# CAMMA-public/SelfPose3d

Measured on AMD Instinct MI355X. Metric: multi-view samples/sec (5-view Panoptic, 80x80x20 voxel), higher is better.
Workload: dtype f32

## Files before the change

include/sp3d.h:

```cpp
#ifndef SP3D_H
#define SP3D_H

#include <stdint.h>

#ifdef __cplusplus
extern "C" {
#endif

#define SP3D_ABI_VERSION 3
#define SP3D_MAX_VIEWS 16
#define SP3D_MAX_TOPK 32

#define SP3D_CAM_STRIDE 64
#define SP3D_CAM_R 0
#define SP3D_CAM_T 9
#define SP3D_CAM_F 12
#define SP3D_CAM_C 14
#define SP3D_CAM_K 16
#define SP3D_CAM_P 19
#define SP3D_CAM_A 21
#define SP3D_CAM_W0 27
#define SP3D_CAM_H0 28
#define SP3D_CAM_FLIP 29
#define SP3D_CAM_RXY 32
// ... 119 lines not shown
                              float beta, void *stream);

int sp3d_channel_shift_act(float *y, const float *shift, const float *residual, int mode, int64_t batch, int C,
                           int64_t inner, int channels_last, void *stream);

int sp3d_fetch_ring(const float *ring, float *dst, uint32_t *counter, int R, int n, void *stream);

int sp3d_maxpool2x_cl(const float *x, float *y, int B, int X, int Y, int Z, int C, void *stream);

int sp3d_crop_shift_act_cl(const float *src, float *dst, const float *shift, int B, int C, int X, int Y, int Z, int SX, int SY,
                           int SZ, int relu, void *stream);

int sp3d_rfft3d(const float *in, float *out, int batch, int SX, int SY, int SZ, void *stream);
int sp3d_irfft3d(float *in, float *out, int batch, int SX, int SY, int SZ, void *stream);

int sp3d_cfft2d(float *data, int batch, int SX, int SY, int inverse, void *stream);
int sp3d_cfft2d_ex(float *data, int batch, int SX, int SY, int inverse, int rows_in, int rows_out, void *stream);

int sp3d_zdft_fwd_cl(const float *x, float *spec, int B, int C, int Cout, int X, int Y, int Z, int SX, int SY, int SZ,
                     void *stream);
int sp3d_zdft_inv_cl(const float *spec, float *y, const float *shift, int B, int O, int X, int Y, int Z, int SX, int SY, int SZ,
                     int relu, void *stream);

int sp3d_unproject_fwd_zdft(const float *const *hm_views, int Jp, const float *cam, const float *centers,
                            const uint8_t *valid, float *spec, int B, int V, int J, int h, int w, int X, int Y, int Z,
                            const float grid_size[3], int W_in, int H_in, int SZ, void *stream);
int sp3d_cfft2d_88_tiled(const float *tiled, float *planes, int batch, int X, int Y, void *stream);

int sp3d_freq_contract_ty(const float *X, const float *T, const float *tw, float *Y, int B, int C, int O, int rows, int SY,
                          void *stream);

int sp3d_gaussian_target_3d(const float *roots, int B, int R, const float *gx, const float *gy, const float *gz, int X,
                            int Y, int Z, float sigma, float *target, void *stream);
int sp3d_render_root_heatmaps(const float *roots, int B, int R, const float *cam, int V, int h, int w, float stride,
                              float *out, void *stream);
int sp3d_render_joints_fwd(const float *kps, const int *count, int N, int P, int J, int h, int w, float sigma, float *out,
                           void *stream);
int sp3d_render_joints_bwd(const float *kps, const int *count, const float *grad_out, int N, int P, int J, int h, int w,
                           float sigma, float *grad_kps, void *stream);

int sp3d_freq_contract(const float *X, const float *W, float *Y, int B, int C, int O, int64_t F, void *stream);
int sp3d_freq_contract_ex(const float *P, const float *Q, float *Y, int I, int J, int K, int64_t F, int64_t sPi,
                          int64_t sPk, int64_t sQj, int64_t sQk, int conj_p, int conj_q, void *stream);

int sp3d_wino_input(const float *x, float *V, int B, int X, int Y, int Z, int C, void *stream);
int sp3d_wino_output(const float *M, float *y, const float *shift, const float *residual, int mode, int B, int X, int Y,
                     int Z, int O, void *stream);
int sp3d_wino_fused(const float *x, const float *U, float *y, const float *shift, const float *residual, int mode, int B,
                    int X, int Y, int Z, int C, int O, void *stream);

int sp3d_wino_fused_split(const float *x, const void *U3, float *y, const float *shift, const float *residual, int mode, int B,
                          int X, int Y, int Z, int C, int O, void *stream);

int sp3d_wino_fused_split64(const float *x, const void *U3, float *y, const float *shift, const float *residual, int mode,
                            int B, int X, int Y, int Z, int C, int O, void *stream);

int sp3d_conv3_split(const float *x, const void *W3, float *y, const float *shift, const float *residual, int mode, int B,
                     int X, int Y, int Z, int C, int O, void *stream);


int sp3d_conv3_split_skip(const float *x, const void *W3, float *y, const float *shift, const float *xs, const void *WS,
                          int B, int X, int Y, int Z, int C, int O, int CS, void *stream);

int sp3d_wino_fused_split64_skip(const float *x, const void *U3, float *y, const float *shift, const float *xs, const void *WS,
                                 int B, int X, int Y, int Z, int C, int O, int CS, void *stream);

int sp3d_upsample2x_scatter(const float *G, float *out, const float *shift, const float *skip, int64_t batch, int X, int Y,
                            int Z, int O, void *stream);

int sp3d_upsample2x_scatter_head(const float *G, float *head, const float *shift, const float *skip, const float *wout,
                                 const float *bout, int64_t batch, int X, int Y, int Z, int O, int J, void *stream);

int sp3d_upconv2x_fused(const float *x, const void *w_split, const float *shift, const float *skip, const float *w_out,
                        const float *b_out, float *out, int64_t batch, int X, int Y, int Z, int CIN, int O, int J, void *stream);

#define SP3D_GBN_F32 0
#define SP3D_GBN_F64 1
#define SP3D_GBN_REPLICAS 16
#define SP3D_GBN_PLAIN 0
#define SP3D_GBN_RELU 1
#define SP3D_GBN_ADD_RELU 2
int64_t sp3d_gbn_workspace_bytes(int G, int C);
int sp3d_gbn_forward(const void *x, void *y, int dtype, const int32_t *group_of, const int32_t *group_samples, int N,
                     int64_t S, int C, int G, int G_update, const void *weight, const void *bias, void *running_mean,
                     void *running_var, double eps, double momentum, int mode, const void *residual, void *mean,
                     void *invstd, void *scale, void *shift, double *workspace, void *stream);
int sp3d_gbn_backward(const void *x, const void *dy, void *dx, int dtype, const int32_t *group_of,
                      const int32_t *group_samples, int N, int64_t S, int C, int G, const void *weight, const void *mean,
                      const void *invstd, const void *scale, const void *shift, int mode, const void *y,
                      void *grad_residual, void *grad_weight, void *grad_bias, void *k123, double *workspace, void *stream);

#ifdef __cplusplus
}
#endif
#endif
```

selfpose3d_amd/_lib.py:

```python
from __future__ import annotations

import ctypes as C
import os
from typing import Optional, Sequence

import torch

_HERE = os.path.dirname(os.path.abspath(__file__))
_DEFAULT_LIB_PATH = os.path.join(_HERE, "libsp3d.so")
NOPK_LIB_PATH = os.path.join(_HERE, "libsp3d_nopk.so")
LIB_PATH = os.environ.get("SP3D_LIB_PATH") or _DEFAULT_LIB_PATH

LAYOUT_PLANAR = 0
LAYOUT_NHWC = 1
OUT_CHANNELS_LAST = 0x100
HM_BF16 = 0x200
OUT_BF16 = 0x400
HM_ONE_CHANNEL = 0x800
HM_WIDE_MASK = 0x1000
OUT_ZSPECTRUM = 0x2000
HM_ONE_ZSPECTRUM = 0x4000
SCATTER_AUTO, SCATTER_PER_TAP, SCATTER_MERGE = 0, 2, 3
SCATTER_WIDE = 0x100
MAX_VIEWS = 16
MAX_TOPK = 32
ABI_VERSION = 3

_CTYPES = {"p": C.c_void_p, "i": C.c_int, "l": C.c_int64, "f": C.c_float, "d": C.c_double, "s": C.c_char_p}

SIGNATURES = {
    "sp3d_abi_version": "i:",
    "sp3d_camera_finish": "i: p i",
    "sp3d_error_string": "s: i",
    "sp3d_pack_heatmaps": "i: pp iiiiii p",
    "sp3d_pack_heatmaps_ex": "i: pp iiiiiiii p",
    "sp3d_unproject_fwd": "i: p ii ppppp iiiiiiii p ii p",
    "sp3d_unproject_fwd_indexed": "i: p ii pppppp iiiiiiii p ii p",
    "sp3d_unproject_fwd_strided": "i: p ii pppppp iiiiiiii p ii p",
    "sp3d_unproject_bwd": "i: pppppp iiiiiiii p ii p",
    "sp3d_unproject_bwd_indexed": "i: ppppppp iiiiiiii p ii p",
    "sp3d_unproject_fwd_train": "i: p ii ppppppp iiiiiiii p ii p",
    "sp3d_unproject_bwd_packed": "i: ppppppp iiiiiiiiii p iii p",
    "sp3d_unproject_bwd_packed_det": "i: pppppppp iiiiiiiiii p iii p",
    "sp3d_fixed_to_float": "i: ppp l p",
    "sp3d_unproject_one_fwd_train": "i: p ii ppppppp iiiiiiii p ii p",
    "sp3d_unproject_one_bwd": "i: ppppp l pp iiiiiiii p ii p",
    "sp3d_unproject_one_bwd_det": "i: ppppp l ppp iiiiiiii p ii p",
    "sp3d_nms_topk_workspace_bytes": "l: iiiii",
    "sp3d_nms_topk": "i: p iiiii ppppppp",
    "sp3d_nms_proposals": "i: p iiiii pp f pppppp",
    "sp3d_soft_argmax": "i: ppp ii l f p",
    "sp3d_soft_argmax_grid": "i: ppp iii p ii f p",
    "sp3d_soft_argmax_grid_train": "i: ppp iii pp ii f p",
    "sp3d_soft_argmax_grid_bwd": "i: ppp iii pppp ii f p",
    "sp3d_channel_shift_act": "i: ppp i l i l i p",
    "sp3d_fetch_ring": "i: ppp ii p",
    "sp3d_maxpool2x_cl": "i: pp iiiii p",
    "sp3d_crop_shift_act_cl": "i: ppp iiiiiiiii p",
    "sp3d_rfft3d": "i: pp iiii p",
    "sp3d_irfft3d": "i: pp iiii p",
    "sp3d_cfft2d": "i: p iiii p",
    "sp3d_cfft2d_ex": "i: p iiiiii p",
    "sp3d_zdft_fwd_cl": "i: pp iiiiiiiii p",
    "sp3d_zdft_inv_cl": "i: ppp iiiiiiiii p",
    "sp3d_unproject_fwd_zdft": "i: p i pppp iiiiiiii p iii p",
    "sp3d_cfft2d_88_tiled": "i: pp iii p",
    "sp3d_freq_contract_ty": "i: pppp iiiii p",
    "sp3d_gaussian_target_3d": "i: p ii ppp iii f pp",
    "sp3d_render_root_heatmaps": "i: p ii p iii f pp",
    "sp3d_render_joints_fwd": "i: pp iiiii f pp",
    "sp3d_render_joints_bwd": "i: ppp iiiii f pp",
    "sp3d_freq_contract": "i: ppp iii l p",
    "sp3d_freq_contract_ex": "i: ppp iii lllll ii p",
    "sp3d_wino_input": "i: pp iiiii p",
    "sp3d_wino_output": "i: pppp iiiiii p",
    "sp3d_wino_fused": "i: ppppp iiiiiii p",
# ... 716 lines not shown

def freq_contract_ex(Pf: torch.Tensor, Qf: torch.Tensor, mode: str, *, out: Optional[torch.Tensor] = None) -> torch.Tensor:
    lib = load()
    _require_cuda(Pf, "Pf")
    Pf, Qf = Pf.resolve_conj().contiguous(), Qf.resolve_conj().contiguous()
    if Pf.dtype != torch.complex64 or Qf.dtype != torch.complex64 or Pf.shape[2:] != Qf.shape[2:]:
        raise Sp3dError("freq_contract_ex: complex64 operands with equal frequency shape expected")
    Fn = 1
    for d in Pf.shape[2:]:
        Fn *= int(d)
    p0, p1, q0, q1 = int(Pf.shape[0]), int(Pf.shape[1]), int(Qf.shape[0]), int(Qf.shape[1])
    if mode == "fwd":
        I, K, J = p0, p1, q0
        sPi, sPk, sQj, sQk, cp, cq = p1 * Fn, Fn, q1 * Fn, Fn, 0, 1
        ok = q1 == p1
    elif mode == "dx":
        I, K, J = p0, p1, q1
        sPi, sPk, sQj, sQk, cp, cq = p1 * Fn, Fn, Fn, q1 * Fn, 0, 0
        ok = q0 == p1
    elif mode == "dw":
        I, K, J = p1, p0, q1
        sPi, sPk, sQj, sQk, cp, cq = Fn, p1 * Fn, Fn, q1 * Fn, 1, 0
        ok = q0 == p0
    else:
        raise Sp3dError(f"freq_contract_ex: unknown mode {mode}")
    if not ok:
        raise Sp3dError("freq_contract_ex: contracted dimensions differ")
    Y = _result_dense(out, (I, J) + tuple(Pf.shape[2:]), torch.complex64, Pf.device, "freq_contract_ex")
    check(lib.sp3d_freq_contract_ex(Pf.data_ptr(), Qf.data_ptr(), Y.data_ptr(), I, J, K, Fn, sPi, sPk, sQj, sQk, cp, cq,
                                    _stream(Pf.device)), "sp3d_freq_contract_ex")
    return Y


_WINO_G = ((1.0, 0.0, 0.0), (0.5, 0.5, 0.5), (0.5, -0.5, 0.5), (0.0, 0.0, 1.0))


def wino_weights(w: torch.Tensor) -> torch.Tensor:
    G = torch.tensor(_WINO_G, dtype=torch.float64, device=w.device)
    u = torch.einsum("ai,bj,ck,ozijk->abczo", G, G, G, w.double())
    return u.reshape(64, w.shape[1], w.shape[0]).float().contiguous()


def wino_weights_split(U: torch.Tensor, chunk: int = 8) -> torch.Tensor:
    P, Cc, O = (int(v) for v in U.shape)
    U = U.float()
    hi = U.bfloat16()
    r = U - hi.float()
    mid = r.bfloat16()
    lo = (r - mid.float()).bfloat16()
    pieces = torch.stack([mid, hi, lo], 0).reshape(3, P, Cc // chunk, chunk // 4, 4, O)
    return pieces.permute(1, 2, 3, 5, 0, 4).contiguous()


def conv_weights_split(w: torch.Tensor) -> torch.Tensor:
    O, Cc = int(w.shape[0]), int(w.shape[1])
    taps = int(w.shape[2]) * int(w.shape[3]) * int(w.shape[4])
    pc = wino_weights_split(w.float().permute(4, 3, 2, 1, 0).reshape(taps, Cc, O).contiguous(), 8)
    mid, hi, lo = pc[..., 0, :], pc[..., 1, :], pc[..., 2, :]
    return torch.stack([hi, lo, hi, hi, mid, mid], -2).contiguous()


def conv_weights_split24(w: torch.Tensor) -> torch.Tensor:
    O, Cc = int(w.shape[0]), int(w.shape[1])
    pc = wino_weights_split(w.float().permute(4, 3, 2, 1, 0).reshape(27, Cc, O).contiguous(), 8)
    pc = pc.reshape(27, Cc // 8, 2, O // 32, 32, 3, 4).permute(0, 1, 3, 2, 4, 5, 6)
    hl = torch.stack([pc[..., 1, :], pc[..., 2, :]], -2).reshape(27, Cc // 8, O // 32, 512)
    mid = pc[..., 0, :].reshape(27, Cc // 8, O // 32, 256)
    return torch.cat([hl, mid], -1).contiguous()


def skip_fold_enabled() -> bool:
    return env_switch("SP3D_FOLD_SKIP", True)


def _require_skip(xs: torch.Tensor, skip_w: torch.Tensor, x: torch.Tensor, CS: int, numel: int, who: str):
    _require_cl3d_f32(xs, who)
    if xs.device != x.device or tuple(xs.shape) != (x.shape[0], CS) + tuple(x.shape[2:]):
        raise Sp3dError(f"{who}: xs must be ({x.shape[0]}, {CS}, ...) on the grid and device of x, got {tuple(xs.shape)} on {xs.device}")
    if skip_w.device != x.device or skip_w.dtype != torch.bfloat16 or not skip_w.is_contiguous() or skip_w.numel() != numel:
        raise Sp3dError(f"{who}: skip_w must be the split records of the ({x.shape[1]}, {CS}, 1, 1, 1) weight on {x.device}; got "
                        f"{tuple(skip_w.shape)}, {skip_w.dtype}, {skip_w.device}, contiguous={skip_w.is_contiguous()}")


def conv3_split_(x: torch.Tensor, W3: torch.Tensor, shift: torch.Tensor, mode: int,
                 residual: Optional[torch.Tensor] = None, *, xs: Optional[torch.Tensor] = None,
                 skip_w: Optional[torch.Tensor] = None, out: Optional[torch.Tensor] = None) -> torch.Tensor:
    lib = load()
    _require_cuda(x, "x")
    B, Cc, X, Y, Z = (int(v) for v in x.shape)
    _require_cl3d_f32(x, "conv3_split_")
    O = int(W3.shape[3])
    dev = x.device
    y = _result_cl3d(out, B, O, X, Y, Z, x, "conv3_split_")
    if xs is not None or skip_w is not None:
        if xs is None or skip_w is None or int(mode) != 1 or residual is not None:
            raise Sp3dError("conv3_split_: the folded skip takes xs AND skip_w, mode 1 and no residual")
        CS = 16
        _require_skip(xs, skip_w, x, CS, CS * O * 6, "conv3_split_")
        check(lib.sp3d_conv3_split_skip(x.data_ptr(), W3.data_ptr(), y.data_ptr(), shift.data_ptr(), xs.data_ptr(),
                                        skip_w.data_ptr(), B, X, Y, Z, Cc, O, CS, _stream(dev)), "sp3d_conv3_split_skip")
        return y
    if residual is not None:
        residual = _as_cl3d(residual)
    check(lib.sp3d_conv3_split(x.data_ptr(), W3.data_ptr(), y.data_ptr(), shift.data_ptr(), _opt(residual), int(mode),
                               B, X, Y, Z, Cc, O, _stream(dev)), "sp3d_conv3_split")
    return y


def quarter_direct_enabled() -> bool:
    return env_switch("SP3D_QUARTER_DIRECT", True)


def quarter_direct_covers(B: int, C: int, O: int, X: int, Y: int, Z: int) -> bool:
    blocks = B * (X // 5) * (Y // 5) * (Z // 5)
    return O == 128 and C in (64, 128) and X % 5 == 0 and Y % 5 == 0 and Z % 5 == 0 and blocks <= 64


def conv3_split128_(x: torch.Tensor, W3: torch.Tensor, shift: torch.Tensor, mode: int,
                    residual: Optional[torch.Tensor] = None, *, out: Optional[torch.Tensor] = None) -> torch.Tensor:
    lib = load()
    _require_cuda(x, "x")
    B, Cc, X, Y, Z = (int(v) for v in x.shape)
    _require_cl3d_f32(x, "conv3_split128_")
    O = 128
    if W3.device != x.device or W3.dtype != torch.bfloat16 or not W3.is_contiguous() or tuple(W3.shape) != (27, Cc // 8, O // 32, 768):
        raise Sp3dError(f"conv3_split128_: W3 must be conv_weights_split24 of the ({O}, {Cc}, 3, 3, 3) weight on {x.device}; got "
                        f"{tuple(W3.shape)}, {W3.dtype}, {W3.device}, contiguous={W3.is_contiguous()}")
    out = _result_cl3d(out, B, O, X, Y, Z, x, "conv3_split128_")
    if residual is not None:
        residual = _as_cl3d(residual)
    check(lib.sp3d_conv3_split(x.data_ptr(), W3.data_ptr(), out.data_ptr(), shift.data_ptr(), _opt(residual), int(mode),
                                  B, X, Y, Z, Cc, O, _stream(x.device)), "sp3d_conv3_split")
    return out


def wino_conv3d_(x: torch.Tensor, U: torch.Tensor, shift: torch.Tensor, mode: int,
                 residual: Optional[torch.Tensor] = None, *, out: Optional[torch.Tensor] = None) -> torch.Tensor:
    lib = load()
    _require_cuda(x, "x")
    B, Cc, X, Y, Z = (int(v) for v in x.shape)
    _require_cl3d_f32(x, "wino_conv3d_")
    O = int(U.shape[2])
    if residual is not None:
        residual = _as_cl3d(residual)
    y = _result_cl3d(out, B, O, X, Y, Z, x, "wino_conv3d_")
    T = B * ((X + 1) // 2) * ((Y + 1) // 2) * ((Z + 1) // 2)
    V = torch.empty((64, T, Cc), dtype=torch.float32, device=x.device)
    check(lib.sp3d_wino_input(x.data_ptr(), V.data_ptr(), B, X, Y, Z, Cc, _stream(x.device)), "sp3d_wino_input")
    M = torch.bmm(V, U)
    check(lib.sp3d_wino_output(M.data_ptr(), y.data_ptr(), shift.data_ptr(), _opt(residual), int(mode), B, X, Y, Z, O,
                               _stream(x.device)), "sp3d_wino_output")
    return y


def wino_fused_conv3d_(x: torch.Tensor, U: torch.Tensor, shift: torch.Tensor, mode: int,
                       residual: Optional[torch.Tensor] = None, U3: Optional[torch.Tensor] = None, *,
                       xs: Optional[torch.Tensor] = None, skip_w: Optional[torch.Tensor] = None,
                       out: Optional[torch.Tensor] = None) -> torch.Tensor:
    lib = load()
    _require_cuda(x, "x")
    B, Cc, X, Y, Z = (int(v) for v in x.shape)
    _require_cl3d_f32(x, "wino_fused_conv3d_")
    O = int(U.shape[2])
    y = _result_cl3d(out, B, O, X, Y, Z, x, "wino_fused_conv3d_")
    if xs is not None or skip_w is not None:
        if xs is None or skip_w is None or U3 is None or int(mode) != 1 or residual is not None:
            raise Sp3dError("wino_fused_conv3d_: the folded skip takes U3, xs AND skip_w, mode 1 and no residual")
        CS = 32
        _require_skip(xs, skip_w, x, CS, CS * O * 3, "wino_fused_conv3d_")
        check(lib.sp3d_wino_fused_split64_skip(x.data_ptr(), U3.data_ptr(), y.data_ptr(), shift.data_ptr(), xs.data_ptr(),
                                               skip_w.data_ptr(), B, X, Y, Z, Cc, O, CS, _stream(x.device)),
              "sp3d_wino_fused_split64_skip")
        return y
    if residual is not None:
        residual = _as_cl3d(residual)
    if U3 is None:
        name, weights = "sp3d_wino_fused", U
    else:
        name, weights = ("sp3d_wino_fused_split64" if O == 64 else "sp3d_wino_fused_split"), U3
    check(getattr(lib, name)(x.data_ptr(), weights.data_ptr(), y.data_ptr(), shift.data_ptr(), _opt(residual), int(mode),
                             B, X, Y, Z, Cc, O, _stream(x.device)), name)
    return y


def upconv_weights_split(w_gemm: torch.Tensor) -> torch.Tensor:
    Cc, O = int(w_gemm.shape[0]), int(w_gemm.shape[1]) // 8
    U = w_gemm.float().reshape(Cc, 8 * O // 32, 32).permute(1, 0, 2).contiguous()
    pc = wino_weights_split(U, 8)
    mid, hi, lo = pc[..., 0, :], pc[..., 1, :], pc[..., 2, :]
    return torch.stack([hi, lo, hi, hi, mid, mid], -2).reshape(8, O // 32, Cc // 8, 2, 32, 6, 4).contiguous()


def _require_upconv_split(w_split: torch.Tensor, Cc: int, O: int, x: torch.Tensor):
    if w_split.device != x.device or w_split.dtype != torch.bfloat16 or not w_split.is_contiguous() or \
            w_split.numel() != Cc * 8 * O * 6:
        raise Sp3dError(f"w_split must be upconv_weights_split(w_gemm) of the ({Cc}, {8 * O}) weight on {x.device}; got "
                        f"{tuple(w_split.shape)}, {w_split.dtype}, {w_split.device}, contiguous={w_split.is_contiguous()}")


def upconv_fused_covers(Cc: int, O: int, head: bool) -> bool:
    return env_switch("SP3D_FUSE_UPCONV", True) and (Cc, O, bool(head)) in ((64, 32, True), (128, 64, False))


def upsample2x_(x: torch.Tensor, w_gemm: torch.Tensor, shift: torch.Tensor, skip: torch.Tensor,
                w_split: Optional[torch.Tensor] = None, *, out: Optional[torch.Tensor] = None) -> torch.Tensor:
    lib = load()
    _require_cuda(x, "x")
    B, Cc, X, Y, Z = (int(v) for v in x.shape)
    _require_cl3d_f32(x, "upsample2x_")
    O = int(w_gemm.shape[1]) // 8
    out = _result_cl3d(out, B, O, 2 * X, 2 * Y, 2 * Z, x, "upsample2x_")
    skip = _as_cl3d(skip)
    if w_split is not None and upconv_fused_covers(Cc, O, False):
        _require_upconv_split(w_split, Cc, O, x)
        check(lib.sp3d_upconv2x_fused(x.data_ptr(), w_split.data_ptr(), shift.data_ptr(), skip.data_ptr(), None, None,
                                      out.data_ptr(), B, X, Y, Z, Cc, O, 0, _stream(x.device)), "sp3d_upconv2x_fused")
        return out
    G = torch.matmul(x.permute(0, 2, 3, 4, 1).reshape(-1, Cc), w_gemm)
    check(lib.sp3d_upsample2x_scatter(G.data_ptr(), out.data_ptr(), shift.data_ptr(), skip.data_ptr(), B, X, Y, Z, O,
                                      _stream(x.device)), "sp3d_upsample2x_scatter")
    return out


def upsample2x_head_(x: torch.Tensor, w_gemm: torch.Tensor, shift: torch.Tensor, skip: torch.Tensor, w_out: torch.Tensor,
                     b_out: torch.Tensor, w_split: Optional[torch.Tensor] = None, *,
                     out: Optional[torch.Tensor] = None) -> torch.Tensor:
    lib = load()
    _require_cuda(x, "x")
    B, Cc, X, Y, Z = (int(v) for v in x.shape)
    _require_cl3d_f32(x, "upsample2x_head_")
    O = int(w_gemm.shape[1]) // 8
    J = int(w_out.shape[0])
    skip = _as_cl3d(skip)
# ... 46 lines not shown
```

selfpose3d_amd/csrc/sp3d_wino_fused.hip:

```cpp
#include <hip/hip_runtime.h>
#include <stdint.h>

#include "../../include/sp3d.h"
#include "sp3d_conv3_host.h"
#include "sp3d_split.h"


namespace sp3d {

#ifdef SP3D_WF_TIMELINE
__device__ unsigned long long *g_wf_tl = nullptr;
#define WF_STAMP(slot) do { __builtin_amdgcn_sched_barrier(0); if (tl && lane == 0) tl[slot] = __builtin_readcyclecounter(); __builtin_amdgcn_sched_barrier(0); } while (0)
#else
#define WF_STAMP(slot) do { } while (0)
#endif

constexpr int WF_RX = 10, WF_RY = 10, WF_RZ = 6;
constexpr int WF_VS = 8;
constexpr int WF_ROW = WF_RX * WF_VS + 4;
constexpr int WF_LDS = WF_RY * WF_RZ * WF_ROW;

__device__ constexpr int wf_ta(int r) { return r == 0 ? 0 : (r == 1 ? 1 : (r == 2 ? 2 : 1)); }
__device__ constexpr int wf_tb(int r) { return r == 0 ? 2 : (r == 1 ? 2 : (r == 2 ? 1 : 3)); }
__device__ constexpr float wf_sb(int r) { return r == 1 ? 1.0f : -1.0f; }
// ... 333 lines not shown
                    acc[4 + bc] = __builtin_elementwise_fma(M1, cv, acc[4 + bc]);
                }
            }
        };
        WfB b0[2], b1[2];
        b0[0] = load_b(0, 0);
        b0[1] = load_b(1, 0);
#pragma unroll 1
        for (int jk = 0; jk < 16; jk += 2) {
            step(jk, jk + 1, b0, b1);
            step(jk + 1, (jk + 2) & 15, b1, b0);
        }
    }

    const float sh = shift[t];
    const int yl = oy0 + 2 * h;
    const int64_t obase = ((((int64_t)b * X + ox0) * Y + yl) * Z + oz0) * O + t;
#pragma unroll
    for (int a = 0; a < 8; ++a) {
        float rv[16];
        if (MODE >= 2) {
#pragma unroll
            for (int v = 0; v < 16; ++v) {
                const int dx = 2 * (v & 3) + (a >> 2), dy = 4 * ((v >> 2) & 1) + ((a >> 1) & 1), dz = 2 * (v >> 3) + (a & 1);
                const int xo = min(ox0 + dx, X - 1), yo = min(yl + dy, Y - 1), zo = min(oz0 + dz, Z - 1);
                rv[v] = res[((((int64_t)b * X + xo) * Y + yo) * Z + zo) * O + t];
            }
        }
#pragma unroll
        for (int v = 0; v < 16; ++v) {
            const int dx = 2 * (v & 3) + (a >> 2), dy = 4 * ((v >> 2) & 1) + ((a >> 1) & 1), dz = 2 * (v >> 3) + (a & 1);
            if (ox0 + dx < X && oz0 + dz < Z && yl + dy < Y) {
                const int64_t idx = obase + (((int64_t)dx * Y + dy) * Z + dz) * O;
                float val = acc[a][v] + sh;
                if (MODE == 2) val += rv[v];
                if (MODE >= 1) val = fmaxf(val, 0.0f);
                if (MODE == 3) val += rv[v];
                y[idx] = val;
            }
        }
    }
}

typedef float f32x4 __attribute__((ext_vector_type(4)));
constexpr int W16_RX = 10, W16_RY = 10, W16_RZ = 4, W16_VS = 16;
constexpr int W16_ROW = W16_RX * W16_VS + 4;
constexpr int W16_LDS = W16_RY * W16_RZ * W16_ROW;

__device__ __forceinline__ f32x4 mfma16_bf16(u32x4 a, u32x4 b, f32x4 c)
{
    return __builtin_amdgcn_mfma_f32_16x16x32_bf16(__builtin_bit_cast(bf16x8, a), __builtin_bit_cast(bf16x8, b), c, 0, 0, 0);
}

template <int C, int MODE, int NBW, int KS, bool SKIP = false>
__global__ __launch_bounds__(64 * (4 / NBW) * KS) __attribute__((amdgpu_waves_per_eu(NBW <= 2 ? 2 : 1))) void wino_fused16_kernel(const float *__restrict__ x,
                                                                          const unsigned *__restrict__ U3,
                                                                          float *__restrict__ y, const float *__restrict__ shift,
                                                                          const float *__restrict__ res, int B, int X, int Y,
                                                                          int Z, int NBX, int NBY, int NBZ,
                                                                          const float *__restrict__ xs = nullptr,
                                                                          const unsigned *__restrict__ WS = nullptr)
{
    constexpr int O = 64, NCH = C / 16, NOW = 4 / NBW, NTG = 64 * NOW;
    static_assert(NCH % KS == 0, "chunks must divide evenly over the channel groups");
    __shared__ __attribute__((aligned(16))) float lds[KS * W16_LDS];
    const int tid = threadIdx.x, lane = tid & 63, wave = tid >> 6;
    const int kg = wave / NOW, ow = wave % NOW, tg = tid - kg * NTG;
    float *region = lds + kg * W16_LDS;
    const int tl = lane & 15, q = lane >> 4;
    int bid = blockIdx.x;
    const int bz = bid % NBZ; bid /= NBZ;
    const int by = bid % NBY; bid /= NBY;
    const int bx = bid % NBX;
    const int b = bid / NBX;
    const int ttx = tl & 3, tty = tl >> 2;
    const int ox0 = bx * 8, oy0 = by * 8, oz0 = bz * 2;
    const float *rb = region + (2 * tty) * W16_ROW + (2 * ttx) * W16_VS + 4 * q;

    f32x4 acc[8][NBW];
#pragma unroll
    for (int a = 0; a < 8; ++a)
#pragma unroll
        for (int n = 0; n < NBW; ++n) acc[a][n] = f32x4{0.0f, 0.0f, 0.0f, 0.0f};
#ifdef SP3D_W16_SETPRIO
    __builtin_amdgcn_s_setprio(SP3D_W16_SETPRIO);
#endif

    constexpr int NV4 = W16_RX * W16_RY * W16_RZ * 4, PER = (NV4 + NTG - 1) / NTG;
    int goff[PER], loff[PER];
#pragma unroll
    for (int u = 0; u < PER; ++u) {
        const int idx = tg + u * NTG;
        const int v = idx >> 2, part = idx & 3;
        const int vx = v % W16_RX, vy = (v / W16_RX) % W16_RY, vz = v / (W16_RX * W16_RY);
        const int gx = ox0 - 1 + vx, gy = oy0 - 1 + vy, gz = oz0 - 1 + vz;
        const bool in = idx < NV4 && gx >= 0 && gx < X && gy >= 0 && gy < Y && gz >= 0 && gz < Z;
        goff[u] = in ? (int)(((((int64_t)gx) * Y + gy) * Z + gz) * C + part * 4) : -1;
        loff[u] = idx < NV4 ? (vz * W16_RY + vy) * W16_ROW + vx * W16_VS + part * 4 : -1;
    }
    const float *xb = x + (int64_t)b * X * Y * Z * C;
    float4 pre[PER];
    auto fetch = [&](int cc) {
#pragma unroll
        for (int u = 0; u < PER; ++u) {
            pre[u] = make_float4(0.0f, 0.0f, 0.0f, 0.0f);
            if (goff[u] >= 0) pre[u] = *reinterpret_cast<const float4 *>(xb + goff[u] + cc * 16);
        }
    };
    fetch(kg);
#pragma unroll 1
    for (int cc = kg; cc < NCH; cc += KS) {
        __syncthreads();
#pragma unroll
        for (int u = 0; u < PER; ++u)
            if (loff[u] >= 0) *reinterpret_cast<float4 *>(region + loff[u]) = pre[u];
        __syncthreads();
        if (cc + KS < NCH) fetch(cc + KS);
        const unsigned *ub = U3 + ((((int64_t)cc * 4 + q) * O) + ow * NBW * 16 + tl) * 6;
        auto load_b = [&](int i, int jk, int n) {
            const unsigned *r = ub + (int64_t)(i * 16 + jk) * NCH * 4 * O * 6 + n * 16 * 6;
            WfB w;
            w.mh = *reinterpret_cast<const u32x4_a8 *>(r);
            w.l = *reinterpret_cast<const u32x2_a8 *>(r + 4);
            return w;
        };
#pragma unroll 1
        for (int jk = 0; jk < 16; ++jk) {
            const int j = jk >> 2, k = jk & 3;
            WfB bw[NBW][4];
#pragma unroll
            for (int n = 0; n < NBW; ++n)
#pragma unroll
                for (int i = 0; i < 4; ++i) {
#if SP3D_W16_ABLATE & 2
                    bw[n][i].mh = u32x4{0x3f803f80u + (unsigned)(jk + n), 0x3f803f80u, 0x3f803f80u + (unsigned)i, 0x3f803f80u};
                    bw[n][i].l = u32x2{0x3f803f80u, 0x3f803f80u};
#else
                    bw[n][i] = load_b(i, jk, n);
#endif
                }
            const int ya = (j == 0) ? 0 : ((j == 2) ? 2 : 1), yb = (j == 3) ? 3 : ((j == 2) ? 1 : 2);
            const int za = (k == 0) ? 0 : ((k == 2) ? 2 : 1), zb = (k == 3) ? 3 : ((k == 2) ? 1 : 2);
            const float sy = (j == 1) ? 1.0f : -1.0f, sz = (k == 1) ? 1.0f : -1.0f;
            const float *r00 = rb + (za * W16_RY + ya) * W16_ROW, *r10 = rb + (za * W16_RY + yb) * W16_ROW;
            const float *r01 = rb + (zb * W16_RY + ya) * W16_ROW, *r11 = rb + (zb * W16_RY + yb) * W16_ROW;
            float g[4][4];
#pragma unroll
            for (int xi = 0; xi < 4; ++xi) {
#if SP3D_W16_ABLATE & 8
                const float f0 = __int_as_float(0x3f800000 + jk + xi), f1 = __int_as_float(0x3f900000 + lane);
                const float4 v00 = make_float4(f0, f1, f0, f1), v10 = make_float4(f1, f0, f1, f0), v01 = v00, v11 = v10;
                (void)r00; (void)r10; (void)r01; (void)r11;
#else
                const float4 v00 = *reinterpret_cast<const float4 *>(r00 + xi * W16_VS), v10 = *reinterpret_cast<const float4 *>(r10 + xi * W16_VS);
                const float4 v01 = *reinterpret_cast<const float4 *>(r01 + xi * W16_VS), v11 = *reinterpret_cast<const float4 *>(r11 + xi * W16_VS);
#endif
                g[xi][0] = fmaf(sz, fmaf(sy, v11.x, v01.x), fmaf(sy, v10.x, v00.x));
                g[xi][1] = fmaf(sz, fmaf(sy, v11.y, v01.y), fmaf(sy, v10.y, v00.y));
                g[xi][2] = fmaf(sz, fmaf(sy, v11.z, v01.z), fmaf(sy, v10.z, v00.z));
                g[xi][3] = fmaf(sz, fmaf(sy, v11.w, v01.w), fmaf(sy, v10.w, v00.w));
            }
            float cyz[4];
#pragma unroll
            for (int bc = 0; bc < 4; ++bc) {
                const int bb = bc >> 1, c2 = bc & 1;
                const float cy = bb == 0 ? (j < 3 ? 1.0f : 0.0f) : (j == 0 ? 0.0f : (j == 1 ? 1.0f : -1.0f));
                const float cz = c2 == 0 ? (k < 3 ? 1.0f : 0.0f) : (k == 0 ? 0.0f : (k == 1 ? 1.0f : -1.0f));
                cyz[bc] = cy * cz;
            }
            f32x4 M0[NBW], M1[NBW];
#pragma unroll
            for (int n = 0; n < NBW; ++n) { M0[n] = f32x4{0.0f, 0.0f, 0.0f, 0.0f}; M1[n] = f32x4{0.0f, 0.0f, 0.0f, 0.0f}; }
#pragma unroll
            for (int i = 0; i < 4; ++i) {
                float av[4];
#pragma unroll
                for (int kk = 0; kk < 4; ++kk)
                    av[kk] = (i == 1) ? g[1][kk] + g[2][kk] : ((i == 3) ? g[3][kk] - g[1][kk] : g[wf_ta(i)][kk] - g[wf_tb(i)][kk]);
                const unsigned hi01 = pack_bf16(av[0], av[1]), hi23 = pack_bf16(av[2], av[3]);
#if SP3D_W16_ABLATE & 4
                const unsigned mid01 = hi01, mid23 = hi23, lo01 = hi01, lo23 = hi23;
#else
                const float r0 = av[0] - bf16_lo(hi01), r1 = av[1] - bf16_hi(hi01), r2 = av[2] - bf16_lo(hi23), r3 = av[3] - bf16_hi(hi23);
                const unsigned mid01 = pack_bf16(r0, r1), mid23 = pack_bf16(r2, r3);
                const unsigned lo01 = pack_bf16(r0 - bf16_lo(mid01), r1 - bf16_hi(mid01));
                const unsigned lo23 = pack_bf16(r2 - bf16_lo(mid23), r3 - bf16_hi(mid23));
#endif
                const u32x4 Qhh = {hi01, hi23, hi01, hi23}, Qmm = {mid01, mid23, mid01, mid23}, Qlh = {lo01, lo23, hi01, hi23};
#pragma unroll
                for (int n = 0; n < NBW; ++n) {
                    const WfB &w = bw[n][i];
                    const u32x4 Bmh = w.mh;
                    const u32x4 Bhl = {w.mh.z, w.mh.w, w.l.x, w.l.y};
#if SP3D_W16_ABLATE & 1
                    {
                        const unsigned z = (Qhh.x ^ Bmh.x) + (Qmm.y ^ Bmh.z) + (Qlh.x ^ Bhl.w) + (Qlh.z ^ Bhl.y);
                        M0[n].x += __uint_as_float(z & 0x3fffffffu);
                        M1[n].y += __uint_as_float((z >> 1) & 0x3fffffffu);
                        continue;
                    }
#endif
                    if (i < 3) {
                        M0[n] = mfma16_bf16(Qhh, Bmh, M0[n]);
                        M0[n] = mfma16_bf16(Qmm, Bmh, M0[n]);
                        M0[n] = mfma16_bf16(Qlh, Bhl, M0[n]);
                    }
                    if (i == 1 || i == 3) {
                        M1[n] = mfma16_bf16(Qhh, Bmh, M1[n]);
                        M1[n] = mfma16_bf16(Qmm, Bmh, M1[n]);
                        M1[n] = mfma16_bf16(Qlh, Bhl, M1[n]);
                    }
                    if (i == 2) {
                        const u32x4 nmh = Bmh ^ 0x80008000u, nhl = Bhl ^ 0x80008000u;
                        M1[n] = mfma16_bf16(Qhh, nmh, M1[n]);
                        M1[n] = mfma16_bf16(Qmm, nmh, M1[n]);
                        M1[n] = mfma16_bf16(Qlh, nhl, M1[n]);
                    }
                }
            }
#pragma unroll
            for (int n = 0; n < NBW; ++n)
#pragma unroll
                for (int bc = 0; bc < 4; ++bc) {
#if defined(SP3D_NO_PK) || defined(SP3D_W16_SCALAR_ACC)
                    for (int e = 0; e < 4; ++e) {
                        acc[bc][n][e] = fmaf(M0[n][e], cyz[bc], acc[bc][n][e]);
                        acc[4 + bc][n][e] = fmaf(M1[n][e], cyz[bc], acc[4 + bc][n][e]);
                    }
#else
                    const f32x4 cv = {cyz[bc], cyz[bc], cyz[bc], cyz[bc]};
                    acc[bc][n] = __builtin_elementwise_fma(M0[n], cv, acc[bc][n]);
                    acc[4 + bc][n] = __builtin_elementwise_fma(M1[n], cv, acc[4 + bc][n]);
#endif
                }
        }
    }

    if (SKIP) {
        constexpr int CS = 32;
        static_assert(!SKIP || KS * 16 == CS, "one skip chunk per channel group");
        int ln = lane;
        asm volatile("" : "+v"(ln));
        const int stl = ln & 15, sq = ln >> 4;
        const float *xsb = xs + (int64_t)b * X * Y * Z * CS + 16 * kg + 4 * sq;
// ... 117 lines not shown
using namespace sp3d;

static int wino_fused_check(const void *x, const void *U, const void *y, const void *shift, const void *residual, int mode, int B,
                            int X, int Y, int Z, bool supported, const Conv3Grid &g)
{
    return conv3_check(B, X, Y, Z, mode, x && U && y && shift && (mode < 2 || residual), supported, g.blocks <= 0x7fffffff);
}

extern "C" int sp3d_wino_fused(const float *x, const float *U, float *y, const float *shift, const float *residual, int mode,
                               int B, int X, int Y, int Z, int C, int O, void *stream)
{
    const Conv3Grid g = conv3_grid(B, X, Y, Z, 8, 8, 4);
    if (const int rc = wino_fused_check(x, U, y, shift, residual, mode, B, X, Y, Z, O == 32 && (C == 16 || C == 32), g)) return rc;
    auto launch = [&](auto c, auto m) {
        hipLaunchKernelGGL((wino_fused_kernel<decltype(c)::value, decltype(m)::value>), dim3((unsigned)g.blocks), dim3(64), 0,
                           (hipStream_t)stream, x, U, y, shift, residual, B, X, Y, Z, g.NBX, g.NBY, g.NBZ);
    };
    with_mode(mode, [&](auto m) { if (C == 16) launch(int_c<16>{}, m); else launch(int_c<32>{}, m); });
    return launch_status();
}

extern "C" int sp3d_debug_wino_fused_timeline(void *dev_buffer)
{
#ifdef SP3D_WF_TIMELINE
    unsigned long long *p = (unsigned long long *)dev_buffer;
    return (int)hipMemcpyToSymbol(HIP_SYMBOL(sp3d::g_wf_tl), &p, sizeof(p));
#else
    (void)dev_buffer;
    return SP3D_EUNSUPPORTED;
#endif
}

extern "C" int sp3d_wino_fused_split(const float *x, const void *U3, float *y, const float *shift, const float *residual, int mode,
                                     int B, int X, int Y, int Z, int C, int O, void *stream)
{
    const Conv3Grid g = conv3_grid(B, X, Y, Z, 8, 8, 4);
    const bool supported = O == 32 && (C == 16 || C == 32) && !(reinterpret_cast<uintptr_t>(U3) & 7);
    if (const int rc = wino_fused_check(x, U3, y, shift, residual, mode, B, X, Y, Z, supported, g)) return rc;
    auto launch = [&](auto c, auto m) {
        hipLaunchKernelGGL((wino_fused3_kernel<decltype(c)::value, decltype(m)::value>), dim3((unsigned)g.blocks), dim3(64), 0,
                           (hipStream_t)stream, x, reinterpret_cast<const unsigned *>(U3), y, shift, residual, B, X, Y, Z, g.NBX,
                           g.NBY, g.NBZ);
    };
    with_mode(mode, [&](auto m) { if (C == 16) launch(int_c<16>{}, m); else launch(int_c<32>{}, m); });
    return launch_status();
}

constexpr int W16_NBW = 2, W16_KS = 2;

extern "C" int sp3d_wino_fused_split64(const float *x, const void *U3, float *y, const float *shift, const float *residual,
                                       int mode, int B, int X, int Y, int Z, int C, int O, void *stream)
{
    const Conv3Grid g = conv3_grid(B, X, Y, Z, 8, 8, 2);
    const bool supported = O == 64 && (C == 32 || C == 64) && !(reinterpret_cast<uintptr_t>(U3) & 7);
    if (const int rc = wino_fused_check(x, U3, y, shift, residual, mode, B, X, Y, Z, supported, g)) return rc;
    auto launch = [&](auto c, auto m) {
        hipLaunchKernelGGL((wino_fused16_kernel<decltype(c)::value, decltype(m)::value, W16_NBW, W16_KS>), dim3((unsigned)g.blocks),
                           dim3(64 * (4 / W16_NBW) * W16_KS), 0, (hipStream_t)stream, x, reinterpret_cast<const unsigned *>(U3), y,
                           shift, residual, B, X, Y, Z, g.NBX, g.NBY, g.NBZ, (const float *)nullptr, (const unsigned *)nullptr);
    };
    with_mode(mode, [&](auto m) { if (C == 32) launch(int_c<32>{}, m); else launch(int_c<64>{}, m); });
    return launch_status();
}

extern "C" int sp3d_wino_fused_split64_skip(const float *x, const void *U3, float *y, const float *shift, const float *xs,
                                            const void *WS, int B, int X, int Y, int Z, int C, int O, int CS, void *stream)
{
    const Conv3Grid g = conv3_grid(B, X, Y, Z, 8, 8, 2);
    const bool supported = O == 64 && C == 64 && CS == 32 && !((reinterpret_cast<uintptr_t>(U3) | reinterpret_cast<uintptr_t>(WS)) & 7) &&
                           !(reinterpret_cast<uintptr_t>(xs) & 15);
    const bool in_range = (int64_t)X * Y * Z * CS <= 0x7fffffff && g.blocks <= 0x7fffffff;
    if (const int rc = conv3_check(B, X, Y, Z, 1, x && U3 && y && shift && xs && WS, supported, in_range)) return rc;
    hipLaunchKernelGGL((wino_fused16_kernel<64, 1, W16_NBW, W16_KS, true>), dim3((unsigned)g.blocks),
                       dim3(64 * (4 / W16_NBW) * W16_KS), 0, (hipStream_t)stream, x, reinterpret_cast<const unsigned *>(U3), y,
                       shift, (const float *)nullptr, B, X, Y, Z, g.NBX, g.NBY, g.NBZ, xs, reinterpret_cast<const unsigned *>(WS));
    return launch_status();
}
```

selfpose3d_amd/v2v_net.py:

```python
from __future__ import annotations

from typing import NamedTuple, Optional

import torch
import torch.nn as nn
import torch.nn.functional as F


def _bn(c):
    from .grouped_bn import GroupedBatchNorm3d
    return GroupedBatchNorm3d(c)


def _grouped(bn, training: bool) -> bool:
    return training and getattr(bn, "groups", None) is not None


def fft_len(n: int) -> int:
    m = n + (n & 1)
    while True:
        r, odd = m, 0
        for q in (2, 3, 5, 7, 11, 13):
            if q > 2 and r % q == 0:
                odd += 1
# ... 151 lines not shown
class Up2x3d(nn.Module):

    def __init__(self, cin, cout):
        super().__init__()
        self.block = nn.Sequential(nn.ConvTranspose3d(cin, cout, 2, stride=2, padding=0, output_padding=0), _bn(cout),
                                   nn.ReLU(True))

    def forward(self, x):
        if _grouped(self.block[1], self.training):
            return self.block[1].grouped_forward(self.block[0](x), relu=True)
        return self.block(x)


class _EncDec(nn.Module):

    def __init__(self):
        super().__init__()
        self.encoder_res1 = Residual3d(32, 64)
        self.encoder_res2 = Residual3d(64, 128)
        self.mid_res = Residual3d(128, 128)
        self.decoder_res2 = Residual3d(128, 128)
        self.decoder_upsample2 = Up2x3d(128, 64)
        self.decoder_res1 = Residual3d(64, 64)
        self.decoder_upsample1 = Up2x3d(64, 32)
        self.skip_res1 = Residual3d(32, 32)
        self.skip_res2 = Residual3d(64, 64)

    def forward(self, x):
        s1 = self.skip_res1(x)
        x = self.encoder_res1(F.max_pool3d(x, 2, 2))
        s2 = self.skip_res2(x)
        x = self.encoder_res2(F.max_pool3d(x, 2, 2))
        x = self.decoder_res2(self.mid_res(x))
        x = self.decoder_upsample2(x) + s2
        x = self.decoder_upsample1(self.decoder_res1(x)) + s1
        return x


class TiledZSpectrum:

    def __init__(self, spec: torch.Tensor, X: int, Y: int, Z: int, SZ: int):
        self.spec, self.X, self.Y, self.Z, self.SZ = spec, int(X), int(Y), int(Z), int(SZ)
        self.shape = (int(spec.shape[0]), int(spec.shape[1]), self.X, self.Y, self.Z)
        self.device, self.is_cuda, self.dtype = spec.device, spec.is_cuda, torch.float32


class _Conv(NamedTuple):
    w: torch.Tensor
    shift: torch.Tensor
    u: Optional[torch.Tensor] = None
    split: Optional[torch.Tensor] = None
    direct: Optional[torch.Tensor] = None
    direct24: Optional[torch.Tensor] = None


class _Res(NamedTuple):
    c1: _Conv
    c2: _Conv
    skip: Optional[torch.Tensor]
    skip_direct: Optional[torch.Tensor] = None
    skip_split: Optional[torch.Tensor] = None


class _Up(NamedTuple):
    wT: torch.Tensor
    shift: torch.Tensor
    wg: torch.Tensor
    split: Optional[torch.Tensor] = None


class _FoldedV2V:

    def __init__(self, net: "V2VNet"):
        self.net = net
        self.key = None
        self.layers = {}
        self.spectra = {}
        self.xpad = {}

    def graph_tensors(self):
        return dict(self.layers), dict(self.spectra), dict(self.xpad)

    @staticmethod
    def _key(net):
        ps = list(net.parameters()) + list(net.buffers())
        w3 = net.front_layers[1].res_branch[0].weight
        return (tuple((p.data_ptr(), p._version) for p in ps), str(w3.device), bool(is_cl(w3)))

    def _ensure_built(self):
        key = self._key(self.net)
        if key != self.key:
            self._build()
            self.key = key

    @staticmethod
    def _fold(conv, bn, transposed=False):
        s = bn.weight / torch.sqrt(bn.running_var + bn.eps)
        shape = (1, -1, 1, 1, 1) if transposed else (-1, 1, 1, 1, 1)
        w = conv.weight * s.view(shape)
        fmt = torch.channels_last_3d if is_cl(conv.weight) else torch.contiguous_format
        b = conv.bias if conv.bias is not None else torch.zeros_like(bn.running_mean)
        return w.contiguous(memory_format=fmt), ((b - bn.running_mean) * s + bn.bias).contiguous()

    @staticmethod
    def _conv3_routes(cin, cout):
        return {conv3_route(cin, cout, s, True, ws, dc) for s in ((1, 2, 2, 2), (1 << 20, 2, 2, 2), (1, 5, 5, 5))
                for ws in (True, False) for dc in (True, False)}

    @staticmethod
    def _conv3_record(w, shift):
        from . import _lib
        cout, cin = int(w.shape[0]), int(w.shape[1])
        routes = _FoldedV2V._conv3_routes(cin, cout)
        if not w.is_cuda or routes == {"library"}:
            return _Conv(w, shift)
        u = _lib.wino_weights(w)
        split = _lib.wino_weights_split(u, 16 if cout == 64 else 8) if "wino_fused_conv3d_" in routes else None
        direct = _lib.conv_weights_split(w) if "conv3_split_" in routes else None
        direct24 = _lib.conv_weights_split24(w) if "conv3_split128_" in routes else None
        return _Conv(w, shift, u, split, direct, direct24)

    def _build(self):
        from . import _lib
        n, layers = self.net, {}
        layers["front"] = _Conv(*self._fold(n.front_layers[0].block[0], n.front_layers[0].block[1]))
        ed = n.encoder_decoder
        for name in ("front_res", "encoder_res1", "encoder_res2", "mid_res", "decoder_res2", "decoder_res1", "skip_res1",
                     "skip_res2"):
            blk = n.front_layers[1] if name == "front_res" else getattr(ed, name)
            w1, s1 = self._fold(blk.res_branch[0], blk.res_branch[1])
            w2, s2 = self._fold(blk.res_branch[3], blk.res_branch[4])
            ws = sd = sp = None
            if len(blk.skip_con) > 0:
                ws, ss = self._fold(blk.skip_con[0], blk.skip_con[1])
                s2 = (s2 + ss).contiguous()
                co, ci = int(ws.shape[0]), int(ws.shape[1])
                if ws.is_cuda and (co, ci) == (32, 16):
                    sd = _lib.conv_weights_split(ws)
                if ws.is_cuda and (co, ci) == (64, 32):
                    sp = _lib.wino_weights_split(ws.reshape(co, ci).t().reshape(1, ci, co).contiguous(), 16)
            layers[name] = _Res(self._conv3_record(w1, s1), self._conv3_record(w2, s2), ws, sd, sp)
        for name in ("decoder_upsample2", "decoder_upsample1"):
            blk = getattr(ed, name).block
            wT, sT = self._fold(blk[0], blk[1], transposed=True)
            wg = wT.permute(0, 2, 3, 4, 1).reshape(wT.shape[0], 8 * wT.shape[1]).contiguous()
            fused = wg.is_cuda and (int(wT.shape[0]), int(wT.shape[1])) in ((128, 64), (64, 32))
            layers[name] = _Up(wT, sT, wg, _lib.upconv_weights_split(wg) if fused else None)
        self.layers, self.spectra, self.xpad = layers, {}, {}

    def _route(self, x, c: "_Conv") -> str:
        from . import _lib
        n = self.net
        if c.u is None or not is_cl(x):
            return "library"
        return conv3_route(int(c.w.shape[1]), int(c.w.shape[0]), (x.shape[0],) + tuple(x.shape[2:]), n.winograd,
                           getattr(n, "wino_split", True), getattr(n, "direct_conv", True),
                           quarter_direct=c.direct24 is not None and _lib.quarter_direct_enabled())

    def _conv3(self, x, c: "_Conv", mode, residual=None, xs=None, skip_w=None):
        from . import _lib
        route = self._route(x, c)
        split = getattr(self.net, "wino_split", True)
        if route == "conv3_split_":
            return _lib.conv3_split_(x, c.direct, c.shift, mode, residual, xs=xs, skip_w=skip_w)
        if route == "wino_fused_conv3d_":
            return _lib.wino_fused_conv3d_(x, c.u, c.shift, mode, residual, c.split if split else None, xs=xs, skip_w=skip_w)
        assert xs is None and skip_w is None, route
        if route == "conv3_split128_":
            return _lib.conv3_split128_(x, c.direct24, c.shift, mode, residual)
        if route == "wino_conv3d_":
            return _lib.wino_conv3d_(x, c.u, c.shift, mode, residual)
        return _lib.channel_shift_act_(F.conv3d(x, c.w, None, 1, 1), c.shift, mode, residual)

    def _folded_skip(self, x, h, r: "_Res"):
        from . import _lib
        if r.skip is None or not _lib.skip_fold_enabled() or not (is_cl(x) and x.is_cuda and x.dtype == torch.float32):
            return None
        route, widths = self._route(h, r.c2), (int(r.c2.w.shape[1]), int(r.c2.w.shape[0]), int(x.shape[1]))
        if route == "conv3_split_" and widths == (32, 32, 16):
            return r.skip_direct
        if route == "wino_fused_conv3d_" and getattr(self.net, "wino_split", True) and widths == (64, 64, 32):
            return r.skip_split
        return None

    def _res(self, x, name):
        r = self.layers[name]
        h = self._conv3(x, r.c1, 1)
        if r.skip is None:
            return self._conv3(h, r.c2, 2, x)
        rec = self._folded_skip(x, h, r)
        if rec is not None:
            return self._conv3(h, r.c2, 1, xs=x, skip_w=rec)
        return self._conv3(h, r.c2, 2, self._conv1(x, r.skip))

    _tuned_shapes: "set[tuple]" = set()
    _tune_gemms = None

    @staticmethod
    def _tunable():
        from . import _lib
        on = _FoldedV2V._tune_gemms
        if on is None:
            on = _lib.env_switch("SP3D_TUNE_GEMM", False)
        return getattr(torch.cuda, "tunable", None) if on else None

    def _run_tuned(self, x):
        tun = self._tunable()
        if tun is None or not x.is_cuda:
            return self._run(x)
        capturing = torch.cuda.is_current_stream_capturing()
        shape_key = (tuple(x.shape), str(x.device), bool(self.net.winograd), bool(self.net.fft_front))
        was_on, was_tuning = tun.is_enabled(), tun.tuning_is_enabled()
        try:
            tun.enable(True)
            first = shape_key not in _FoldedV2V._tuned_shapes and not capturing
            tun.tuning_enable(bool(first))
            if first:
                tun.set_max_tuning_duration(30)
            out = self._run(x)
# ... 289 lines not shown
```

Baseline: 2946.

## Add 2D Winograd (YZ-only) variant of fused split-bf16 conv3 kernel for 64-channel layers

Adds a Winograd variant that transforms only the Y and Z axes (48 transformed weight slices) and treats X as a direct 3-tap correlation inside the MFMA loop. The input X transform is dropped, and each X input plane feeds two output accumulators through the three X-tap weights. The host precomputes the YZ-transformed split weights and routes 64-output-channel layers to the new path by default, including the folded-skip variant. This removes X-axis transform arithmetic and its rounding error, at the cost of more MFMA work per tile than full 3D Winograd and extra weight memory.

```diff
diff --git a/include/sp3d.h b/include/sp3d.h
--- a/include/sp3d.h
+++ b/include/sp3d.h
@@ -195,6 +195,7 @@
 int sp3d_wino_fused_split(const float *x, const void *U3, float *y, const float *shift, const float *residual, int mode, int B,
                           int X, int Y, int Z, int C, int O, void *stream);
 
+#define SP3D_CONV3_WINO_YZ 0x100
 int sp3d_wino_fused_split64(const float *x, const void *U3, float *y, const float *shift, const float *residual, int mode,
                             int B, int X, int Y, int Z, int C, int O, void *stream);
 
diff --git a/selfpose3d_amd/_lib.py b/selfpose3d_amd/_lib.py
--- a/selfpose3d_amd/_lib.py
+++ b/selfpose3d_amd/_lib.py
@@ -22,6 +22,7 @@
 HM_ONE_ZSPECTRUM = 0x4000
 SCATTER_AUTO, SCATTER_PER_TAP, SCATTER_MERGE = 0, 2, 3
 SCATTER_WIDE = 0x100
+CONV3_WINO_YZ = 0x100
 MAX_VIEWS = 16
 MAX_TOPK = 32
 ABI_VERSION = 3
@@ -844,6 +845,20 @@
     return pieces.permute(1, 2, 3, 5, 0, 4).contiguous()
 
 
+def wino_yz_weights(w: torch.Tensor) -> torch.Tensor:
+    G = torch.tensor(_WINO_G, dtype=torch.float64, device=w.device)
+    u = torch.einsum("bj,ck,ozijk->ibczo", G, G, w.double())
+    return u.reshape(48, w.shape[1], w.shape[0]).float().contiguous()
+
+
+def wino_yz_weights_split(w: torch.Tensor) -> torch.Tensor:
+    return wino_weights_split(wino_yz_weights(w), 16)
+
+
+def wino_yz_enabled() -> bool:
+    return env_switch("SP3D_WINO_YZ", True)
+
+
 def conv_weights_split(w: torch.Tensor) -> torch.Tensor:
     O, Cc = int(w.shape[0]), int(w.shape[1])
     taps = int(w.shape[2]) * int(w.shape[3]) * int(w.shape[4])
@@ -948,20 +963,26 @@
 def wino_fused_conv3d_(x: torch.Tensor, U: torch.Tensor, shift: torch.Tensor, mode: int,
                        residual: Optional[torch.Tensor] = None, U3: Optional[torch.Tensor] = None, *,
                        xs: Optional[torch.Tensor] = None, skip_w: Optional[torch.Tensor] = None,
-                       out: Optional[torch.Tensor] = None) -> torch.Tensor:
+                       U3yz: Optional[torch.Tensor] = None, out: Optional[torch.Tensor] = None) -> torch.Tensor:
     lib = load()
     _require_cuda(x, "x")
     B, Cc, X, Y, Z = (int(v) for v in x.shape)
     _require_cl3d_f32(x, "wino_fused_conv3d_")
     O = int(U.shape[2])
     y = _result_cl3d(out, B, O, X, Y, Z, x, "wino_fused_conv3d_")
+    yz = 0
+    if U3yz is not None and U3 is not None and O == 64 and wino_yz_enabled():
+        if U3yz.device != x.device or U3yz.dtype != torch.bfloat16 or not U3yz.is_contiguous() or U3yz.numel() != 48 * Cc * O * 3:
+            raise Sp3dError(f"wino_fused_conv3d_: U3yz must be wino_yz_weights_split of the ({O}, {Cc}, 3, 3, 3) weight on {x.device}; "
+                            f"got {tuple(U3yz.shape)}, {U3yz.dtype}, {U3yz.device}, contiguous={U3yz.is_contiguous()}")
+        U3, yz = U3yz, CONV3_WINO_YZ
     if xs is not None or skip_w is not None:
         if xs is None or skip_w is None or U3 is None or int(mode) != 1 or residual is not None:
             raise Sp3dError("wino_fused_conv3d_: the folded skip takes U3, xs AND skip_w, mode 1 and no residual")
         CS = 32
         _require_skip(xs, skip_w, x, CS, CS * O * 3, "wino_fused_conv3d_")
         check(lib.sp3d_wino_fused_split64_skip(x.data_ptr(), U3.data_ptr(), y.data_ptr(), shift.data_ptr(), xs.data_ptr(),
-                                               skip_w.data_ptr(), B, X, Y, Z, Cc, O, CS, _stream(x.device)),
+                                               skip_w.data_ptr(), B, X, Y, Z, Cc, O, CS | yz, _stream(x.device)),
               "sp3d_wino_fused_split64_skip")
         return y
     if residual is not None:
@@ -970,7 +991,7 @@
         name, weights = "sp3d_wino_fused", U
     else:
         name, weights = ("sp3d_wino_fused_split64" if O == 64 else "sp3d_wino_fused_split"), U3
-    check(getattr(lib, name)(x.data_ptr(), weights.data_ptr(), y.data_ptr(), shift.data_ptr(), _opt(residual), int(mode),
+    check(getattr(lib, name)(x.data_ptr(), weights.data_ptr(), y.data_ptr(), shift.data_ptr(), _opt(residual), int(mode) | yz,
                              B, X, Y, Z, Cc, O, _stream(x.device)), name)
     return y
 
diff --git a/selfpose3d_amd/csrc/sp3d_wino_fused.hip b/selfpose3d_amd/csrc/sp3d_wino_fused.hip
--- a/selfpose3d_amd/csrc/sp3d_wino_fused.hip
+++ b/selfpose3d_amd/csrc/sp3d_wino_fused.hip
@@ -409,7 +409,7 @@
     return __builtin_amdgcn_mfma_f32_16x16x32_bf16(__builtin_bit_cast(bf16x8, a), __builtin_bit_cast(bf16x8, b), c, 0, 0, 0);
 }
 
-template <int C, int MODE, int NBW, int KS, bool SKIP = false>
+template <int C, int MODE, int NBW, int KS, bool SKIP = false, bool XD = false>
 __global__ __launch_bounds__(64 * (4 / NBW) * KS) __attribute__((amdgpu_waves_per_eu(NBW <= 2 ? 2 : 1))) void wino_fused16_kernel(const float *__restrict__ x,
                                                                           const unsigned *__restrict__ U3,
                                                                           float *__restrict__ y, const float *__restrict__ shift,
@@ -484,11 +484,12 @@
 #pragma unroll 1
         for (int jk = 0; jk < 16; ++jk) {
             const int j = jk >> 2, k = jk & 3;
-            WfB bw[NBW][4];
+            constexpr int NXP = XD ? 3 : 4;
+            WfB bw[NBW][NXP];
 #pragma unroll
             for (int n = 0; n < NBW; ++n)
 #pragma unroll
-                for (int i = 0; i < 4; ++i) {
+                for (int i = 0; i < NXP; ++i) {
 #if SP3D_W16_ABLATE & 2
                     bw[n][i].mh = u32x4{0x3f803f80u + (unsigned)(jk + n), 0x3f803f80u, 0x3f803f80u + (unsigned)i, 0x3f803f80u};
                     bw[n][i].l = u32x2{0x3f803f80u, 0x3f803f80u};
@@ -533,7 +534,8 @@
                 float av[4];
 #pragma unroll
                 for (int kk = 0; kk < 4; ++kk)
-                    av[kk] = (i == 1) ? g[1][kk] + g[2][kk] : ((i == 3) ? g[3][kk] - g[1][kk] : g[wf_ta(i)][kk] - g[wf_tb(i)][kk]);
+                    av[kk] = XD ? g[i][kk]
+                                : ((i == 1) ? g[1][kk] + g[2][kk] : ((i == 3) ? g[3][kk] - g[1][kk] : g[wf_ta(i)][kk] - g[wf_tb(i)][kk]));
                 const unsigned hi01 = pack_bf16(av[0], av[1]), hi23 = pack_bf16(av[2], av[3]);
 #if SP3D_W16_ABLATE & 4
                 const unsigned mid01 = hi01, mid23 = hi23, lo01 = hi01, lo23 = hi23;
@@ -544,9 +546,26 @@
                 const unsigned lo23 = pack_bf16(r2 - bf16_lo(mid23), r3 - bf16_hi(mid23));
 #endif
                 const u32x4 Qhh = {hi01, hi23, hi01, hi23}, Qmm = {mid01, mid23, mid01, mid23}, Qlh = {lo01, lo23, hi01, hi23};
+                if (XD) {
+#pragma unroll
+                    for (int n = 0; n < NBW; ++n)
+#pragma unroll
+                        for (int e = 0; e < 2; ++e) {
+                            const int dx = i - e;
+                            if (dx < 0 || dx > 2) continue;
+                            const WfB &w = bw[n][dx < NXP ? dx : 0];
+                            const u32x4 Bmh = w.mh;
+                            const u32x4 Bhl = {w.mh.z, w.mh.w, w.l.x, w.l.y};
+                            f32x4 &M = e ? M1[n] : M0[n];
+                            M = mfma16_bf16(Qhh, Bmh, M);
+                            M = mfma16_bf16(Qmm, Bmh, M);
+                            M = mfma16_bf16(Qlh, Bhl, M);
+                        }
+                    continue;
+                }
 #pragma unroll
                 for (int n = 0; n < NBW; ++n) {
-                    const WfB &w = bw[n][i];
+                    const WfB &w = bw[n][i < NXP ? i : 0];
                     const u32x4 Bmh = w.mh;
                     const u32x4 Bhl = {w.mh.z, w.mh.w, w.l.x, w.l.y};
 #if SP3D_W16_ABLATE & 1
@@ -770,14 +789,20 @@
                                        int mode, int B, int X, int Y, int Z, int C, int O, void *stream)
 {
     const Conv3Grid g = conv3_grid(B, X, Y, Z, 8, 8, 2);
+    const bool yz = mode >= 0 && (mode & SP3D_CONV3_WINO_YZ);
+    if (yz) mode &= ~SP3D_CONV3_WINO_YZ;
     const bool supported = O == 64 && (C == 32 || C == 64) && !(reinterpret_cast<uintptr_t>(U3) & 7);
     if (const int rc = wino_fused_check(x, U3, y, shift, residual, mode, B, X, Y, Z, supported, g)) return rc;
-    auto launch = [&](auto c, auto m) {
-        hipLaunchKernelGGL((wino_fused16_kernel<decltype(c)::value, decltype(m)::value, W16_NBW, W16_KS>), dim3((unsigned)g.blocks),
-                           dim3(64 * (4 / W16_NBW) * W16_KS), 0, (hipStream_t)stream, x, reinterpret_cast<const unsigned *>(U3), y,
-                           shift, residual, B, X, Y, Z, g.NBX, g.NBY, g.NBZ, (const float *)nullptr, (const unsigned *)nullptr);
+    auto launch = [&](auto c, auto m, auto xd) {
+        hipLaunchKernelGGL((wino_fused16_kernel<decltype(c)::value, decltype(m)::value, W16_NBW, W16_KS, false, decltype(xd)::value>),
+                           dim3((unsigned)g.blocks), dim3(64 * (4 / W16_NBW) * W16_KS), 0, (hipStream_t)stream, x,
+                           reinterpret_cast<const unsigned *>(U3), y, shift, residual, B, X, Y, Z, g.NBX, g.NBY, g.NBZ,
+                           (const float *)nullptr, (const unsigned *)nullptr);
     };
-    with_mode(mode, [&](auto m) { if (C == 32) launch(int_c<32>{}, m); else launch(int_c<64>{}, m); });
+    with_mode(mode, [&](auto m) {
+        if (yz) { if (C == 32) launch(int_c<32>{}, m, std::true_type{}); else launch(int_c<64>{}, m, std::true_type{}); }
+        else { if (C == 32) launch(int_c<32>{}, m, std::false_type{}); else launch(int_c<64>{}, m, std::false_type{}); }
+    });
     return launch_status();
 }
 
@@ -785,12 +810,17 @@
                                             const void *WS, int B, int X, int Y, int Z, int C, int O, int CS, void *stream)
 {
     const Conv3Grid g = conv3_grid(B, X, Y, Z, 8, 8, 2);
+    const bool yz = CS >= 0 && (CS & SP3D_CONV3_WINO_YZ);
+    if (yz) CS &= ~SP3D_CONV3_WINO_YZ;
     const bool supported = O == 64 && C == 64 && CS == 32 && !((reinterpret_cast<uintptr_t>(U3) | reinterpret_cast<uintptr_t>(WS)) & 7) &&
                            !(reinterpret_cast<uintptr_t>(xs) & 15);
     const bool in_range = (int64_t)X * Y * Z * CS <= 0x7fffffff && g.blocks <= 0x7fffffff;
     if (const int rc = conv3_check(B, X, Y, Z, 1, x && U3 && y && shift && xs && WS, supported, in_range)) return rc;
-    hipLaunchKernelGGL((wino_fused16_kernel<64, 1, W16_NBW, W16_KS, true>), dim3((unsigned)g.blocks),
-                       dim3(64 * (4 / W16_NBW) * W16_KS), 0, (hipStream_t)stream, x, reinterpret_cast<const unsigned *>(U3), y,
-                       shift, (const float *)nullptr, B, X, Y, Z, g.NBX, g.NBY, g.NBZ, xs, reinterpret_cast<const unsigned *>(WS));
+    auto launch = [&](auto xd) {
+        hipLaunchKernelGGL((wino_fused16_kernel<64, 1, W16_NBW, W16_KS, true, decltype(xd)::value>), dim3((unsigned)g.blocks),
+                           dim3(64 * (4 / W16_NBW) * W16_KS), 0, (hipStream_t)stream, x, reinterpret_cast<const unsigned *>(U3), y,
+                           shift, (const float *)nullptr, B, X, Y, Z, g.NBX, g.NBY, g.NBZ, xs, reinterpret_cast<const unsigned *>(WS));
+    };
+    if (yz) launch(std::true_type{}); else launch(std::false_type{});
     return launch_status();
 }
diff --git a/selfpose3d_amd/v2v_net.py b/selfpose3d_amd/v2v_net.py
--- a/selfpose3d_amd/v2v_net.py
+++ b/selfpose3d_amd/v2v_net.py
@@ -227,6 +227,7 @@
     split: Optional[torch.Tensor] = None
     direct: Optional[torch.Tensor] = None
     direct24: Optional[torch.Tensor] = None
+    split_yz: Optional[torch.Tensor] = None
 
 
 class _Res(NamedTuple):
@@ -293,7 +294,8 @@
         split = _lib.wino_weights_split(u, 16 if cout == 64 else 8) if "wino_fused_conv3d_" in routes else None
         direct = _lib.conv_weights_split(w) if "conv3_split_" in routes else None
         direct24 = _lib.conv_weights_split24(w) if "conv3_split128_" in routes else None
-        return _Conv(w, shift, u, split, direct, direct24)
+        split_yz = _lib.wino_yz_weights_split(w) if split is not None and cout == 64 else None
+        return _Conv(w, shift, u, split, direct, direct24, split_yz)
 
     def _build(self):
         from . import _lib
@@ -339,7 +341,8 @@
         if route == "conv3_split_":
             return _lib.conv3_split_(x, c.direct, c.shift, mode, residual, xs=xs, skip_w=skip_w)
         if route == "wino_fused_conv3d_":
-            return _lib.wino_fused_conv3d_(x, c.u, c.shift, mode, residual, c.split if split else None, xs=xs, skip_w=skip_w)
+            return _lib.wino_fused_conv3d_(x, c.u, c.shift, mode, residual, c.split if split else None, xs=xs, skip_w=skip_w,
+                                           U3yz=c.split_yz if split else None)
         assert xs is None and skip_w is None, route
         if route == "conv3_split128_":
             return _lib.conv3_split128_(x, c.direct24, c.shift, mode, residual)
```

Result: faster. 3007 (median of 6 runs) (+2.1%).
